# tdj28/ml-depth-pro-video

Measured on AMD Instinct MI355X. Metric: frames/sec at 1536x1536 (1/2/4/8 MI355X) + depth L1 vs reference, higher is better.
Workload: dtype bf16+f16; 1 GPU; BASELINE config 2/3: one 1536x1536 frame per GPU per step through DepthPro.infer (patch+image+FOV ViT-L, decoder, heads), hipGraph replay; global_batch=1, parallelism=frame-dp1, graph=True

## Files before the change

### ml-depth-pro-video_amd/csrc/dp_gemm.hip

```cpp
#include "dp_gemm_impl.h"

namespace dpg {
std::atomic<int> g_dbg_flags{0};

constexpr int DP_MAX_DEV = 64;
std::atomic<int> g_num_cu[DP_MAX_DEV];
int num_cus() {
  int dev = 0;
  if (hipGetDevice(&dev) != hipSuccess || dev < 0) dev = 0;
  std::atomic<int>& slot = g_num_cu[dev < DP_MAX_DEV ? dev : 0];
  int n = slot.load(std::memory_order_relaxed);
  if (n <= 0) {
    if (hipDeviceGetAttribute(&n, hipDeviceAttributeMultiprocessorCount, dev) != hipSuccess || n <= 0) n = 256;
    if (dev < DP_MAX_DEV) slot.store(n, std::memory_order_relaxed);
  }
  return n;
}
}

namespace {
int launch_tile(const GemmP& p, int tile, bool conv, bool bf16, hipStream_t s) {
  switch (tile) {
    case DP_TILE_PBIG_320x256: case DP_TILE_PBIG_256x256: return launch_part_pbig(p, tile, conv, bf16, s);
    case DP_TILE_256x64: case DP_TILE_256x32: case DP_TILE_128x128: case DP_TILE_DUAL_256x128:
      return launch_part_small(p, tile, conv, bf16, s);
    case DP_TILE_8PH_256x256: case DP_TILE_P8PH_256x256: return launch_part_8ph(p, tile, conv, bf16, s);
    case DP_TILE_8PH_320x256: return launch_part_8ph320(p, conv, bf16, s);
    case DP_TILE_CV3_256x256: return launch_part_cv3(p, conv, bf16, s);
    case DP_TILE_CV3_192x256: return launch_part_cv3(p, conv, bf16, s, 12);
    case DP_TILE_CV3_384x128: return launch_part_cv3(p, conv, bf16, s, 24);
    case DP_TILE_BIG_320x256: case DP_TILE_BIG_512x128: return launch_part_big320(p, tile, conv, bf16, s);
    default: return launch_part_big(p, tile, conv, bf16, s);
  }
}
}


extern "C" int dp_gemm_debug_flags(int flags) {
  g_dbg_flags.store(flags, std::memory_order_relaxed);
  return 0;
}

extern "C" int64_t dp_gemm_workspace_size(void) { return SK_FLAG_BYTES + (int64_t)SK_MAX_WG * SK_TILE_F * 4; }

namespace {
__global__ void ws_check_kernel(uint32_t* __restrict__ ws, int32_t* __restrict__ status) {
  const uint32_t err = ws[DP_GEMM_WS_ERROR_OFFSET / 4];
  if (threadIdx.x == 0) status[0] = (int32_t)err;
  if (err == 0) return;
  __syncthreads();
  for (int i = threadIdx.x; i < (int)(SK_FLAG_BYTES / 4); i += blockDim.x) ws[i] = 0u;
}
}

extern "C" int dp_gemm_workspace_check(void* workspace, int32_t* status, dp_stream_t stream) {
  if (!workspace || !status) return DP_ERR_ARG;
  hipLaunchKernelGGL(ws_check_kernel, dim3(1), dim3(256), 0, (hipStream_t)stream, (uint32_t*)workspace, status);
  DP_CHECK_LAUNCH();
  return 0;
}

namespace {
int gemm_plan(const dp_gemm_args* a, GemmP& p, int& tile) {
  if (!a) return DP_ERR_ARG;
  if (a->M <= 0 || a->N <= 0 || a->K <= 0) return DP_ERR_SHAPE;
  if (a->K % BK != 0 || a->N % 4 != 0) return DP_ERR_SHAPE;
  if (a->ldb % 8 != 0 || (a->a_mode == DP_A_DENSE && a->lda % 8 != 0)) return DP_ERR_ALIGN;
  if ((!a->head_w && a->store_mode != DP_STORE_HEAD_PS && a->ldc % 4 != 0) || (a->R1 && a->ldr1 % 4 != 0) ||
      (a->R2 && a->ldr2 % 4 != 0) || (a->pos && a->ldpos % 4 != 0))
    return DP_ERR_ALIGN;
  if (!a->A || !a->B || (!a->C && !a->ln_xl)) return DP_ERR_ARG;
  if (a->dtype != DP_BF16 && a->dtype != DP_F16) return DP_ERR_DTYPE;
  if (a->c_dtype != DP_BF16 && a->c_dtype != DP_F16 && a->c_dtype != DP_F32) return DP_ERR_DTYPE;
  if (a->c_dtype != DP_F32 && a->c_dtype != a->dtype) return DP_ERR_DTYPE;
  if (a->accumulate && a->c_dtype != DP_F32) return DP_ERR_DTYPE;
  if (a->pos && (a->pos_group <= 0)) return DP_ERR_ARG;
  if (a->a_mode == DP_A_CONV) {
    if (a->in_c % BK != 0 || a->k_h * a->k_w * a->in_c != a->K) return DP_ERR_SHAPE;
    if (a->out_h <= 0 || a->out_w <= 0 || a->stride <= 0 || a->M % (a->out_h * a->out_w) != 0)
      return DP_ERR_SHAPE;
  }
  if (a->store_mode == DP_STORE_HEAD_PS) {
    if (a->a_mode != DP_A_CONV || a->N != 128 || !a->head_w || !a->head_corr || a->c_dtype != DP_F32 ||
        a->accumulate || a->R1 || a->R2 || a->pos || a->gamma || a->act != DP_ACT_NONE)
      return DP_ERR_ARG;
  }
  if (a->store_mode == DP_STORE_ROWS && a->head_corr) {
    if (a->a_mode != DP_A_CONV || a->k_h != 3 || a->k_w != 3 || a->pad != 1 || a->stride != 1 || a->head_w ||
        a->relu_a ||
        a->row_group || a->out_h != a->in_h || a->out_w != a->in_w || a->N % 8 != 0 || a->N < 128 ||
        (a->tile != DP_TILE_AUTO && a->tile <= DP_TILE_256x32))
      return DP_ERR_ARG;
  }
  if (a->store_mode == DP_STORE_DECONV2X2) {
    if (a->dc_cout % 4 != 0 || a->N != 4 * a->dc_cout || a->dc_h <= 0 || a->dc_w <= 0 ||
        a->M % (a->dc_h * a->dc_w) != 0)
      return DP_ERR_SHAPE;
  }
  const bool lnp = a->ln_part_out || a->ln_xb_out || a->ln_xl || a->ln_rs_out,
             lnc = a->ln_part_in || a->ln_colsum || a->ln_rs_in;
  if (lnp && lnc) return DP_ERR_ARG;
  if (lnp && !a->ln_xl && (!a->ln_part_out || !a->ln_xb_out || !a->accumulate || !a->C || a->c_dtype != DP_F32 ||
                           a->act != DP_ACT_NONE || a->N % 128 != 0))
    return DP_ERR_ARG;
  if (a->ln_xl && (!a->ln_xb_out || !a->accumulate || a->c_dtype != DP_F32 || a->act != DP_ACT_NONE ||
                   a->N % 128 != 0 || a->ldc % 8 != 0 || (long long)a->M * a->ldc * 4 >= 0xFFFFFF00LL))
    return DP_ERR_ARG;
  if (lnc && (!(a->ln_part_in || a->ln_rs_in) || (a->ln_part_in && a->ln_rs_in) || !a->ln_colsum || a->K != 1024 ||
              a->accumulate || a->c_dtype == DP_F32 || a->gamma || (a->act != DP_ACT_NONE && a->act != DP_ACT_GELU) ||
              !(a->ln_eps > 0.f)))
    return DP_ERR_ARG;
  if (a->ln_rs_out && (!a->ln_xl || !a->ln_part_out || a->N != 1024 || !(a->ln_eps > 0.f) ||
                       !(a->workspace && a->workspace_bytes >= dp_gemm_workspace_size()) ||
                       (a->M + 319) / 320 > 1023 - LN_CNT_WORD))
    return DP_ERR_ARG;
  if (a->ln_rs_in && a->tile != DP_TILE_AUTO && a->tile != DP_TILE_P8PH_256x256) return DP_ERR_ARG;
  if ((lnp || lnc) && a->tile != DP_TILE_AUTO && a->tile != DP_TILE_8PH_320x256 &&
      !(lnc && a->tile == DP_TILE_P8PH_256x256))
    return DP_ERR_ARG;
  const bool ws_ok = a->workspace && a->workspace_bytes >= dp_gemm_workspace_size();
  const int dbg = g_dbg_flags.load(std::memory_order_relaxed);
  tile = a->tile;
  if (a->store_mode == DP_STORE_HEAD_PS) {
    if (tile != DP_TILE_CV3_256x256 && tile != DP_TILE_CV3_384x128 && tile != DP_TILE_BIG_256x128)
      tile = a->M >= 512 * 256 ? DP_TILE_BIG_512x128 : DP_TILE_BIG_256x128;
  } else if (a->head_w) {
    if (a->N > 32 || a->store_mode != DP_STORE_ROWS) return DP_ERR_SHAPE;
    tile = DP_TILE_256x32;
  }
  const bool col8_shape = a->N % 8 == 0 && !(a->store_mode == DP_STORE_DECONV2X2 && a->dc_cout % 8 != 0);
  const bool col8_align = !(a->c_dtype != DP_F32 && a->ldc % 8 != 0) && !(a->R1 && a->ldr1 % 8 != 0) &&
                          !(a->R2 && a->ldr2 % 8 != 0);
  if (tile >= DP_TILE_BIG_256x256) {
    if (!col8_shape) return DP_ERR_SHAPE;
    if (!col8_align) return DP_ERR_ALIGN;
  }
  const long long tiles256 = (long long)((a->M + 255) / 256) * (a->N / 256);
  if (tile == DP_TILE_STREAMK_256x256 && (!ws_ok || a->N % 256 != 0)) return DP_ERR_ARG;
  if (tile == DP_TILE_AUTO) {
    if (a->N <= 32) tile = DP_TILE_256x32;
    else if (a->N <= 64) tile = DP_TILE_256x64;
    else if (!col8_shape || !col8_align) tile = DP_TILE_128x128;
    else if (a->N == 128 && a->M >= 512 * 256) {
      const bool cv3 = a->a_mode == DP_A_CONV && a->k_h == 3 && a->k_w == 3 && a->stride == 1 && a->pad == 1 &&
                       a->in_h == a->in_w && a->out_h == a->in_h && a->out_w == a->in_w && a->in_w % 16 == 0 &&
                       a->in_c % 64 == 0 && a->head_corr && a->store_mode == DP_STORE_ROWS && a->c_dtype != DP_F32 &&
                       !a->R1 && !a->R2 && !a->gamma && !a->pos && !a->accumulate && !a->row_group && !(dbg & 4096);
      tile = !cv3 ? DP_TILE_BIG_512x128
             : a->in_w % 48 == 0 ? DP_TILE_CV3_384x128 : DP_TILE_CV3_256x256;
    }
    else if (a->N % 256 != 0) tile = DP_TILE_BIG_256x128;
    else if (ws_ok && a->a_mode == DP_A_CONV && !(dbg & 32) && tiles256 < num_cus() &&
             a->K >= 4608) {
      tile = DP_TILE_STREAMK_256x256;
    } else if (ws_ok && a->K <= 256 && tiles256 >= 1024) {
      tile = DP_TILE_STREAMK_256x256;
    } else {
      const long long ncu = num_cus();
      const long long tiles320 = (long long)((a->M + 319) / 320) * (a->N / 256);
      const long long tiles128 = (long long)((a->M + 255) / 256) * (a->N / 128);
      const long long cost256 = (tiles256 + ncu - 1) / ncu * 256 * 20, cost320 = (tiles320 + ncu - 1) / ncu * 320 * 20;
      const long long cost128 = (tiles128 + ncu - 1) / ncu * 128 * 23;
      if (cost128 < cost256 && cost128 < cost320) tile = DP_TILE_BIG_256x128;
      else if (cost320 < cost256) tile = DP_TILE_BIG_320x256;
      else tile = (tiles256 >= 600 && a->a_mode != DP_A_CONV) ? DP_TILE_8PH_256x256 : DP_TILE_BIG_256x256;
      if (tile == DP_TILE_8PH_256x256 && (dbg & 8192)) tile = DP_TILE_BIG_320x256;
      else if (tile == DP_TILE_8PH_256x256 && (dbg & 16384)) tile = DP_TILE_BIG_256x256;
    }
  }
  int ksplit = 1;
  if (tile == DP_TILE_SPLITK_256x256) {
    if (!ws_ok || a->N % 256 != 0 || a->store_mode != DP_STORE_ROWS || a->row_group || a->head_w || a->head_corr ||
        lnp || lnc)
      return DP_ERR_ARG;
    const long long ncu = num_cus(), kt = a->K / BK;
    const long long slab = (long long)a->M * a->N * 4;
    long long sp = ncu / tiles256;
    if (sp > kt / 2) sp = kt / 2;
    if (sp > (a->workspace_bytes - SK_FLAG_BYTES) / slab) sp = (a->workspace_bytes - SK_FLAG_BYTES) / slab;
    if (sp > 32) sp = 32;
    if (sp < 2) return DP_ERR_SHAPE;
    ksplit = (int)sp;
  }
  unsigned c_bytes = 0;
  if (a->store_mode == DP_STORE_ROWS && !a->head_w && !a->head_corr) {
    long long last = a->M - 1;
    if (a->row_group) last = (last / a->row_group) * a->row_group_out + a->row_off + last % a->row_group;
    const long long ext = (last * a->ldc + a->N) * (a->c_dtype == DP_F32 ? 4 : 2);
    if (ext < 0xFFFFFF00LL) c_bytes = (unsigned)ext;
  }
  unsigned dcv_bytes = 0;
  if (a->store_mode == DP_STORE_DECONV2X2 && a->c_dtype != DP_F32) {
    const long long ext = ((4LL * a->M - 1) * a->ldc + a->dc_cout) * 2;
    if (ext < 0xFFFFFF00LL) dcv_bytes = (unsigned)ext;
  }
  const bool off32 = (a->a_mode != DP_A_DENSE || (long long)a->M * a->lda < (1LL << 31)) &&
                     (long long)a->N * a->ldb < (1LL << 31);
  if (!off32) c_bytes = dcv_bytes = 0;
  if ((tile == DP_TILE_PBIG_320x256 || tile == DP_TILE_PBIG_256x256) && (!c_bytes || a->N % 256)) return DP_ERR_ARG;
  if (a->tile == DP_TILE_AUTO && c_bytes && !(dbg & 1024)) {
    const long long ncu = num_cus();
    const bool dense_ok = a->a_mode == DP_A_CONV || (dbg & 2048);
    if (dense_ok && tile == DP_TILE_BIG_320x256 && (long long)((a->M + 319) / 320) * (a->N / 256) >= 2 * ncu)
      tile = DP_TILE_PBIG_320x256;
    else if (dense_ok && tile == DP_TILE_BIG_256x256 && tiles256 >= 2 * ncu)
      tile = DP_TILE_PBIG_256x256;
  }
  const bool dcv = a->store_mode == DP_STORE_DECONV2X2 && !a->relu_a && !a->gamma && a->act == DP_ACT_NONE &&
                   a->dc_w >= 8;
  if (a->tile == DP_TILE_AUTO && dcv && col8_shape && col8_align && !(dbg & (1 << 23)) && tiles256 >= 128)
    tile = DP_TILE_P8PH_256x256;
  if (tile == DP_TILE_P8PH_256x256 || (a->tile == DP_TILE_AUTO && tile == DP_TILE_8PH_256x256 && !(dbg & (1 << 22)))) {
    const bool ok = a->a_mode == DP_A_DENSE && a->N % 256 == 0 && a->K >= 128 && a->c_dtype != DP_F32 &&
                    ((a->store_mode == DP_STORE_ROWS && c_bytes) || (dcv && dcv_bytes)) && !a->R1 && !a->R2 && !a->pos && !a->accumulate &&
                    !a->row_group && !a->head_w && !a->head_corr && !(dbg & (1 << 20));
    if (tile == DP_TILE_P8PH_256x256 && !ok) return DP_ERR_ARG;
    if (ok) tile = DP_TILE_P8PH_256x256;
    if (ok && dcv) c_bytes = dcv_bytes;
  }
  const bool lnc_p8 = lnc && tile == DP_TILE_P8PH_256x256 && (ws_ok || a->ln_rs_in) && !(dbg & (1 << 25)) &&
                      (a->ln_rs_in || (long long)(a->M + 255) / 256 * 256 * 8 <= (long long)SK_TILE_F * 4);
  if (a->ln_rs_in && !lnc_p8) return DP_ERR_ARG;
  if ((lnp || lnc) && !lnc_p8) tile = DP_TILE_8PH_320x256;
  if (tile == DP_TILE_8PH_320x256 || (a->tile == DP_TILE_AUTO && tile == DP_TILE_BIG_320x256 && !(dbg & (1 << 15)))) {
    const bool plain = a->a_mode == DP_A_DENSE && !a->relu_a && a->N % 256 == 0 && a->store_mode == DP_STORE_ROWS &&
                       !a->R1 && !a->R2 && !a->pos && !a->row_group && !a->head_w && !a->head_corr &&
                       !(dbg & (1 << 20)) && off32;
    const bool epi_ok = (!a->accumulate && a->c_dtype != DP_F32) ||
                        (a->accumulate && a->c_dtype == DP_F32 && a->act == DP_ACT_NONE);
    if (tile == DP_TILE_8PH_320x256 && !(plain && epi_ok)) return DP_ERR_ARG;
    if (plain && epi_ok) tile = DP_TILE_8PH_320x256;
  }
  if (a->tile == DP_TILE_AUTO && !(dbg & (1 << 16)) && a->a_mode == DP_A_CONV && a->k_h == 3 && a->k_w == 3 &&
      a->stride == 1 && a->pad == 1 && a->in_h == a->in_w && a->out_h == a->in_h && a->out_w == a->in_w &&
      a->in_w % 16 == 0 && a->in_c % 64 == 0 && a->N % 256 == 0 && a->store_mode == DP_STORE_ROWS &&
      !a->row_group && !a->head_w && !a->head_corr && (long long)a->M * a->in_c < (1LL << 30) && off32 &&
      a->c_dtype != DP_F32 && !a->gamma && !a->pos && !a->accumulate && a->act != DP_ACT_GELU && col8_align &&
      (long long)(a->M / 256) * (a->N / 256) >= 4LL * num_cus())
    tile = DP_TILE_CV3_256x256;
  else if (a->tile == DP_TILE_AUTO && !(dbg & (1 << 16)) && a->a_mode == DP_A_CONV &&
           a->k_h == 3 && a->k_w == 3 && a->stride == 1 && a->pad == 1 && a->in_h == a->in_w &&
           a->out_h == a->in_h && a->out_w == a->in_w && a->in_w % 16 == 0 && a->in_w % 12 == 0 &&
           a->in_c % 64 == 0 && a->N % 256 == 0 && a->store_mode == DP_STORE_ROWS && !a->row_group && !a->head_w &&
           !a->head_corr && (long long)a->M * a->in_c < (1LL << 30) && off32 && a->c_dtype != DP_F32 && !a->gamma &&
           !a->pos && !a->accumulate && a->act != DP_ACT_GELU && col8_align) {
    const long long t12 = (long long)(a->M / ((long long)a->in_w * a->in_w)) * (a->in_w / 12) * (a->in_w / 16) * (a->N / 256);
    const long long ncu = num_cus();
    if (t12 >= 2 * ncu && t12 % ncu == 0 && ((long long)(a->M / 256) * (a->N / 256)) % ncu != 0) tile = DP_TILE_CV3_192x256;
    else if (t12 <= ncu && 2 * t12 >= ncu) tile = DP_TILE_CV3_192x256;
  }
  if (tile >= DP_TILE_BIG_256x256 && !col8_shape) return DP_ERR_SHAPE;
  if (tile >= DP_TILE_BIG_256x256 && !col8_align) return DP_ERR_ALIGN;
  if (tile == DP_TILE_CV3_256x256 || tile == DP_TILE_CV3_192x256 || tile == DP_TILE_CV3_384x128) {
    const int th = tile == DP_TILE_CV3_192x256 ? 12 : tile == DP_TILE_CV3_384x128 ? 24 : 16, S = a->out_w;
    const bool hps = a->store_mode == DP_STORE_HEAD_PS, bc = a->store_mode == DP_STORE_ROWS && a->head_corr;
    if (a->a_mode != DP_A_CONV || a->k_h != 3 || a->k_w != 3 || a->stride != 1 || a->pad != 1 || a->in_h != S ||
        a->in_w != S || a->out_h != S || S % 16 != 0 || S % th != 0 || a->row_group || (a->head_w && !hps) || a->gamma ||
        a->pos || a->accumulate || (a->act != DP_ACT_NONE && a->act != DP_ACT_RELU) ||
        (long long)a->M * a->in_c >= (1LL << 30) || (long long)a->N * a->ldb >= (1LL << 31))
      return DP_ERR_ARG;
    if (!hps && a->store_mode != DP_STORE_ROWS) return DP_ERR_ARG;
    if (bc && (a->c_dtype == DP_F32 || a->R1 || a->R2 || a->N % 128 != 0)) return DP_ERR_ARG;
    if (!hps && !bc && (a->c_dtype == DP_F32 || a->N % 256 != 0)) return DP_ERR_ARG;
    if (th == 12 && (hps || bc)) return DP_ERR_ARG;
    if (th == 24 && !((hps || bc) && a->N == 128)) return DP_ERR_ARG;
  }
  if (a->store_mode == DP_STORE_ROWS && a->head_corr && tile != DP_TILE_BIG_512x128 && tile != DP_TILE_CV3_256x256 &&
      tile != DP_TILE_CV3_384x128)
    return DP_ERR_ARG;
  if (tile == DP_TILE_CV3_384x128 && (!a->head_corr || a->N != 128)) return DP_ERR_ARG;

  p.M = a->M; p.N = a->N; p.K = a->K;
  p.A = (const u16*)a->A; p.lda = a->lda;
  p.B = (const u16*)a->B; p.ldb = a->ldb;
  p.relu_a = a->relu_a;
  p.in_h = a->in_h; p.in_w = a->in_w; p.in_c = a->in_c; p.k_h = a->k_h; p.k_w = a->k_w;
  p.stride = a->stride; p.pad = a->pad; p.out_h = a->out_h; p.out_w = a->out_w;
  p.bias = a->bias; p.act = a->act; p.gamma = a->gamma;
  p.pos = a->pos; p.ldpos = a->ldpos; p.pos_group = a->pos_group; p.pos_off = a->pos_off;
  p.R1 = (const u16*)a->R1; p.ldr1 = a->ldr1; p.R2 = (const u16*)a->R2; p.ldr2 = a->ldr2;
  p.C = a->C; p.ldc = a->ldc; p.c_dtype = a->c_dtype; p.accumulate = a->accumulate;
  p.store_mode = a->store_mode; p.dc_h = a->dc_h; p.dc_w = a->dc_w; p.dc_cout = a->dc_cout;
  p.row_group = a->row_group; p.row_group_out = a->row_group_out; p.row_off = a->row_off;
  p.head_w = a->head_w; p.head_b = a->head_b; p.head_corr = a->head_corr;
  p.ln_part_out = a->ln_part_out; p.ln_xb_out = (u16*)a->ln_xb_out; p.ln_xl = (u16*)a->ln_xl;
  p.ln_part_in = a->ln_part_in; p.ln_colsum = a->ln_colsum; p.ln_eps = a->ln_eps;
  p.ln_rs = a->ln_rs_in;
  p.ln_rs_out = a->ln_rs_out;
  p.ln_cnt = a->ln_rs_out ? (unsigned*)a->workspace + LN_CNT_WORD : nullptr;
  p.tiles_n = 1;
  p.tiles_m = 1;
  if (tile == DP_TILE_STREAMK_256x256) {
    p.tiles_n = a->N / 256;
    p.tiles_m = (a->M + 255) / 256;
  }
  p.dbg = dbg;
  p.c_bytes = c_bytes;
  p.ksplit = ksplit;
  p.kpart = ksplit > 1 ? (float*)((char*)a->workspace + SK_FLAG_BYTES) : nullptr;
  p.groups = 1;
  return 0;
}
}

extern "C" int dp_gemm_plan(const dp_gemm_args* a, int32_t* tile_out, int32_t* grid_out) {
  GemmP p;
  int tile = 0;
  const int rc = gemm_plan(a, p, tile);
  if (rc) return rc;
  const int N = a->N, M = a->M;
  int bm = 256, bn = 128;
  switch (tile) {
    case DP_TILE_256x64: bn = 64; break;
    case DP_TILE_256x32: bn = 32; break;
    case DP_TILE_128x128: bm = 128; bn = 128; break;
    case DP_TILE_BIG_256x128: case DP_TILE_BIG_256x128_K32: case DP_TILE_DEEP_256x128: bn = 128; break;
    case DP_TILE_BIG_320x256: bm = 320; bn = 256; break;
    case DP_TILE_BIG_512x128: bm = 512; bn = 128; break;
    case DP_TILE_DUAL_256x128: bn = 128; break;
    case DP_TILE_PBIG_320x256: case DP_TILE_8PH_320x256: bm = 320; bn = 256; break;
    case DP_TILE_CV3_192x256: bm = 192; bn = 256; break;
    case DP_TILE_CV3_384x128: bm = 384; bn = 128; break;
    default: bn = 256;
  }
  if (tile_out) *tile_out = tile;
  int grid = ((M + bm - 1) / bm) * ((N + bn - 1) / bn);
  if (tile == DP_TILE_PBIG_320x256 || tile == DP_TILE_PBIG_256x256 || tile == DP_TILE_P8PH_256x256)
    grid = grid < num_cus() ? grid : num_cus();
  if (tile == DP_TILE_SPLITK_256x256) grid *= p.ksplit;
  if (grid_out) *grid_out = tile == DP_TILE_STREAMK_256x256 ? sk_grid(p) : grid;
  return 0;
}

extern "C" int dp_gemm(const dp_gemm_args* a, dp_stream_t stream) {
  GemmP p;
  int tile = 0;
  const int rc = gemm_plan(a, p, tile);
  if (rc) return rc;
  hipStream_t s = (hipStream_t)stream;
  const bool conv = a->a_mode == DP_A_CONV;
  if (tile == DP_TILE_STREAMK_256x256) return launch_part_sk(p, conv, a->workspace, a->dtype == DP_BF16, s);
  if (tile == DP_TILE_SPLITK_256x256) return launch_part_splitk(p, conv, a->dtype == DP_BF16, s);
  if (tile == DP_TILE_P8PH_256x256 && a->ln_part_in && !a->ln_rs_in) {
    float* rs = (float*)((char*)a->workspace + SK_FLAG_BYTES);
    hipLaunchKernelGGL(ln_merge_kernel, dim3((a->M + 255) / 256), dim3(256), 0, s, a->ln_part_in, a->M, a->ln_eps, rs);
    DP_CHECK_LAUNCH();
    p.ln_rs = rs;
  }
  return launch_tile(p, tile, conv, a->dtype == DP_BF16, s);
}

extern "C" int dp_gemm_grouped(const dp_gemm_args* a, int32_t groups, dp_stream_t stream) {
  if (!a || groups < 1 || groups > DP_MAX_GROUPS) return DP_ERR_ARG;
  if (groups == 1) return dp_gemm(a, stream);
  GemmP p;
  for (int g = 0; g < groups; ++g) {
    GemmP q;
    int t = 0;
    const int rc = gemm_plan(&a[g], q, t);
    if (rc) return rc;
    const dp_gemm_args &x = a[0], &y = a[g];
    if (y.M != x.M || y.N != x.N || y.K != x.K || y.dtype != x.dtype || y.lda != x.lda || y.ldb != x.ldb ||
        y.a_mode != DP_A_DENSE || x.a_mode != DP_A_DENSE || y.relu_a || y.act != x.act ||
        !y.bias != !x.bias || !y.gamma != !x.gamma || !y.pos != !x.pos || y.ldpos != x.ldpos ||
        y.pos_group != x.pos_group || y.pos_off != x.pos_off || !y.R1 != !x.R1 || y.ldr1 != x.ldr1 ||
        !y.R2 != !x.R2 || y.ldr2 != x.ldr2 || y.ldc != x.ldc || y.c_dtype != x.c_dtype ||
        y.accumulate != x.accumulate || y.store_mode != DP_STORE_ROWS || x.store_mode != DP_STORE_ROWS ||
        y.row_group != x.row_group || y.row_group_out != x.row_group_out || y.row_off != x.row_off ||
        y.head_w || y.head_corr || y.N % 8 != 0 || y.ln_part_out || y.ln_xb_out || y.ln_xl || y.ln_part_in ||
        y.ln_rs_out || y.ln_rs_in ||
        y.ln_colsum)
      return DP_ERR_ARG;
    if (g == 0) p = q;
    p.grp[g] = GemmP::Group{q.A, q.B, q.bias, q.gamma, q.pos, q.R1, q.R2, q.C};
  }
  p.groups = groups;
  hipStream_t s = (hipStream_t)stream;
  return launch_part_big(p, TILE_GRP_128x128, false, a->dtype == DP_BF16, s);
}
```

### ml-depth-pro-video_amd/csrc/dp_gemm_cv3.hip

```cpp
#include "dp_gemm_impl.h"

namespace {

constexpr int CV_TW = 16;
constexpr int CV_PW = CV_TW + 2;
template <int TH> struct CvGeo {
  static constexpr int PIX = (TH + 2) * CV_PW;
  static constexpr int PPW = (PIX * 8 + 511) / 512;
  static constexpr int PATCH_B = 8 * PPW * 1024;
  static constexpr int FM = TH / 2, HQ = FM / 2;
  static constexpr int NREAL = (PIX + 7) / 8;
  static constexpr bool TIGHT = NREAL * 1024 + ((FM + 1) * CV_PW + 2) * 128 < 65536;
  static constexpr int PSTRIDE = TIGHT ? NREAL * 1024 : PATCH_B;
  static constexpr int TRASH = 2 * PSTRIDE;
  static constexpr int WOFF = TIGHT ? 2 * PSTRIDE + 1024 : 2 * PATCH_B;
};

constexpr int CV_EPI_RES = 0, CV_EPI_BC = 1, CV_EPI_HPS = 2;
constexpr int CV_STAMPS = 10, CV_STAMP_WGS = 4096;
__device__ unsigned long long g_cv3_stamp[CV_STAMP_WGS * CV_STAMPS];
template <typename K_, bool RELU, int BN, int EPI, int ABL = 0, int TH = 16>
__global__ void __launch_bounds__(512, 1) gemm_cv3_kernel(const GemmP p) {
  using G = CvGeo<TH>;
  constexpr int FM = G::FM, HQ = G::HQ, PPW = G::PPW, CV_PATCH_B = G::PATCH_B, CV_PIX = G::PIX;
  constexpr bool TIGHT = G::TIGHT;
  constexpr int PSTRIDE = G::PSTRIDE, WOFF = G::WOFF;
  constexpr int TN = BN / 4, FN = TN / 16, QF = FN / 2;
  static_assert(TH == 16 || TH == 12 || (TH == 24 && BN == 128), "tile rows");
  constexpr int NBH = BN / 128;
  constexpr int B_B = BN * 128;
  static_assert(EPI != CV_EPI_RES || BN == 256, "residual epilogue: BN 256");
  static_assert(EPI != CV_EPI_HPS || BN == 128, "head epilogue: one parity (32 columns) per wave");
  __shared__ __attribute__((aligned(1024))) char smem[WOFF + 2 * B_B];

  const int tid = threadIdx.x, lane = tid & 63;
  const int wave = tid >> 6;
  const int wave_u = __builtin_amdgcn_readfirstlane(wave);
  unsigned long long st_[CV_STAMPS] = {};
  if constexpr ((ABL & 8) != 0) { st_[0] = __builtin_amdgcn_s_memtime(); st_[4] = __builtin_amdgcn_s_memrealtime(); }
  const int wm = wave >> 2, wn = wave & 3;
  const int nwg = gridDim.x, bid = blockIdx.x;
  const int xcd = bid & 7, q8 = nwg >> 3, r8 = nwg & 7;
  const int wgid = (xcd < r8 ? xcd * (q8 + 1) : r8 * (q8 + 1) + (xcd - r8) * q8) + (bid >> 3);
  const int S = p.out_w, tpr = S / CV_TW, tpi = (S / TH) * tpr;
  const int tn = wgid % p.tiles_n, sp = wgid / p.tiles_n;
  const int img = sp / tpi, r_ = sp - img * tpi;
  const int y0 = (r_ / tpr) * TH, x0 = (r_ % tpr) * CV_TW, n0 = tn * BN;
  const int cin = p.in_c, CB = cin / 64;
  const int KT = CB * 9;

  constexpr uint32_t CV_PAD = 0x80000000u;
  auto patch_off = [&](int i, int c0) __attribute__((always_inline)) {
    const int c = c0 + i * 64;
    const int P = c >> 3, slot = c & 7;
    uint32_t off = CV_PAD;
    if (P < CV_PIX) {
      const int pr = P / CV_PW, pc = P - pr * CV_PW;
      const int iy = y0 - 1 + pr, ix = x0 - 1 + pc;
      if ((unsigned)iy < (unsigned)S && (unsigned)ix < (unsigned)S)
        off = 2u * (uint32_t)(((img * S + iy) * S + ix) * cin + ((slot ^ (P & 7)) << 3));
    }
    return off;
  };
  const uint32_t lds0 = __builtin_amdgcn_readfirstlane(lds_addr(smem));
  const u32x4_t a_rs = raw_rsrc(p.A, (uint32_t)((long long)p.M * cin * 2));

  constexpr int HALF = 128 * 128;
  const int prow = wave * 8 + (lane >> 3);
  const int pchunk = (lane & 7) ^ ((lane >> 3) & 7);
  const uint32_t boff = 2u * (uint32_t)((n0 + prow) * (int)p.ldb + pchunk * 8);
  auto issue_b = [&](int h, int t) {
    const uint32_t dst = lds0 + WOFF + (t & 1) * B_B + h * HALF + wave_u * 1024;
    #pragma unroll
    for (int i = 0; i < 2; ++i) glds16s(boff, p.B + (long long)(h * 128 + i * 64) * p.ldb + 64 * t, dst + i * 8192);
  };
  auto issue_patch3 = [&](int cb, int buf, int i0) {
    int c0 = wave * PPW * 64 + lane;
    asm volatile("" : "+v"(c0));
    #pragma unroll
    for (int i = i0; i < i0 + PPW / 2; ++i) {
      const int j = wave_u * PPW + i;
      const uint32_t dst = lds0 + ((!TIGHT || j < G::NREAL) ? buf * PSTRIDE + j * 1024 : G::TRASH);
      glds16b(patch_off(i, c0) + cb * 128, a_rs, dst);
    }
  };

  f32x4_t acc[FM][FN];
  #pragma unroll
  for (int i = 0; i < FM; ++i)
    #pragma unroll
    for (int j = 0; j < FN; ++j) acc[i][j] = f32x4_t{0.f, 0.f, 0.f, 0.f};
  const int frow = lane & 15, fchunk = lane >> 4;
  uint4 af[2][HQ], bf[2][2][QF];
  typedef __attribute__((address_space(3))) const char lds_c;
  typedef __attribute__((address_space(3))) const u32x4_t lds_u4;
  uint32_t abase[8][2], bbase[2];
  {
    const int PB = wm * FM * CV_PW + frow;
    #pragma unroll
    for (int v = 0; v < 8; ++v)
      #pragma unroll
      for (int ks = 0; ks < 2; ++ks) abase[v][ks] = lds0 + PB * 128 + (((ks * 4 + fchunk) ^ ((PB + v) & 7)) << 4);
    #pragma unroll
    for (int ks = 0; ks < 2; ++ks)
      bbase[ks] = lds0 + WOFF + (wn * TN + frow) * 128 + (((ks * 4 + fchunk) ^ (frow & 7)) << 4);
  }
  auto readA = [&](int qm, int ky, int kx, int pb) __attribute__((always_inline)) {
    const int boff_ = TIGHT ? pb * PSTRIDE : 0;
    #pragma unroll
    for (int ks = 0; ks < 2; ++ks)
      #pragma unroll
      for (int fm = 0; fm < HQ; ++fm) {
        const int c = (qm * HQ + fm + ky) * CV_PW + kx;
        af[ks][fm] = __builtin_bit_cast(uint4, *(lds_u4*)((lds_c*)(uintptr_t)abase[c & 7][ks] + boff_ + c * 128));
      }
    if constexpr (RELU && (ABL & 32)) {
      #pragma unroll
      for (int ks = 0; ks < 2; ++ks)
        #pragma unroll
        for (int fm = 0; fm < HQ; ++fm) af[ks][fm] = relu_pk16(af[ks][fm]);
      __builtin_amdgcn_sched_barrier(0);
    }
  };
  auto readB = [&](int qn, int st) __attribute__((always_inline)) {
    #pragma unroll
    for (int ks = 0; ks < 2; ++ks)
      #pragma unroll
      for (int fn = 0; fn < QF; ++fn)
        bf[qn][ks][fn] = __builtin_bit_cast(uint4, *(lds_u4*)((lds_c*)(uintptr_t)bbase[ks] + st * B_B + (qn * (TN / 2) + fn * 16) * 128));
  };
  auto tick = [&]() -> unsigned long long {
    if constexpr ((ABL & 256) != 0) return __builtin_amdgcn_s_memtime();
    return 0ull;
  };
  auto mma = [&](int qm, int qn) {
    const unsigned long long m0_ = tick();
    asm volatile("s_waitcnt lgkmcnt(0)" ::: "memory");
    __builtin_amdgcn_sched_barrier(0);
    const unsigned long long m1_ = tick();
    if constexpr ((ABL & 256) != 0) st_[8] += m1_ - m0_;
    if constexpr (ABL & 4) return;
    if constexpr (RELU && !(ABL & 32)) {
      if (qn == 0) {
        #pragma unroll
        for (int ks = 0; ks < 2; ++ks)
          #pragma unroll
          for (int fm = 0; fm < HQ; ++fm) af[ks][fm] = relu_pk16(af[ks][fm]);
      }
    }
    if constexpr ((ABL & 1536) == 0) __builtin_amdgcn_s_setprio(1);
    #pragma unroll
    for (int ks = 0; ks < 2; ++ks)
      #pragma unroll
      for (int fm = 0; fm < HQ; ++fm) {
        #pragma unroll
        for (int fn = 0; fn < QF; ++fn)
          acc[qm * HQ + fm][qn * QF + fn] = K_::mfma16(bf[qn][ks][fn], af[ks][fm], acc[qm * HQ + fm][qn * QF + fn]);
      }
    if constexpr ((ABL & 1536) == 0) __builtin_amdgcn_s_setprio(0);
    if constexpr ((ABL & 256) != 0) { __builtin_amdgcn_sched_barrier(0); st_[9] += tick() - m1_; }
  };
  auto bar = [&]() {
    const unsigned long long b0_ = tick();
    if constexpr ((ABL & 16) == 0) asm volatile("s_barrier" ::: "memory");
    if constexpr ((ABL & 256) != 0) st_[7] += tick() - b0_;
  };

  issue_patch3(0, 0, 0); issue_patch3(0, 0, PPW / 2);
  #pragma unroll
  for (int h = 0; h < NBH; ++h) issue_b(h, 0);
  if (KT > 1) {
    #pragma unroll
    for (int h = 0; h < NBH; ++h) issue_b(h, 1);
    wait_vmcnt<2 * NBH>();
  } else {
    wait_vmcnt<0>();
  }
  lds_barrier();
  if constexpr ((ABL & 8) != 0) st_[1] = __builtin_amdgcn_s_memtime();
  if constexpr ((ABL & 512) != 0) { if (wave_u >= 4) __builtin_amdgcn_s_setprio(1); }
  if (wm == 1) bar();
  int cb = 0;
  auto block = [&](auto st0_tag) __attribute__((always_inline)) {
    constexpr int ST0 = decltype(st0_tag)::value;
    constexpr int pb = ST0;
    const bool nb = cb + 1 < CB;
    #pragma unroll
    for (int tap = 0; tap < 9; ++tap) {
      const int ky = tap / 3, kx = tap - ky * 3, st = (ST0 + tap) & 1;
      const int t = cb * 9 + tap;
      const bool np = tap == 0 && nb;
      const bool n2 = t + 2 < KT;
      readA(0, ky, kx, pb); readB(0, st); readB(1, st);
      if (np && !(ABL & 2) && !(ABL & 128)) { issue_patch3(cb + 1, pb ^ 1, 0); issue_patch3(cb + 1, pb ^ 1, PPW / 2); }
      bar(); mma(0, 0); mma(0, 1); bar();
      readA(1, ky, kx, pb);
      if (n2 && !(ABL & 2) && !(ABL & 64)) issue_b(0, t + 2);
      const unsigned long long v0_ = tick();
      if (np) { if (n2) wait_vmcnt<PPW + 2>(); else wait_vmcnt<PPW>(); }
      else { if (n2) wait_vmcnt<2>(); else wait_vmcnt<0>(); }
      if constexpr ((ABL & 256) != 0) st_[6] += tick() - v0_;
      if (NBH == 2 && n2 && !(ABL & 2) && !(ABL & 64)) issue_b(1, t + 2);
      bar(); mma(1, 0); mma(1, 1); bar();
    }
    if constexpr (!TIGHT) {
      const uint32_t d = pb ? (uint32_t)-CV_PATCH_B : (uint32_t)CV_PATCH_B;
      #pragma unroll
      for (int v = 0; v < 8; ++v)
        #pragma unroll
        for (int ks = 0; ks < 2; ++ks) abase[v][ks] += d;
    }
    ++cb;
  };
  for (int pair = 0; pair < CB / 2; ++pair) {
    block(std::integral_constant<int, 0>{});
    block(std::integral_constant<int, 1>{});
  }
  if (CB & 1) block(std::integral_constant<int, 0>{});
  if (wm == 0) bar();
  if constexpr ((ABL & 512) != 0) __builtin_amdgcn_s_setprio(0);

  lds_barrier();
  if constexpr ((ABL & 8) != 0) st_[2] = __builtin_amdgcn_s_memtime();
  if constexpr ((ABL & 1) != 0) {
    float z = 0.f;
    #pragma unroll
    for (int i = 0; i < FM; ++i)
      #pragma unroll
      for (int j = 0; j < FN; ++j) z += acc[i][j][0];
    if (z == 1234.5f) ((float*)p.C)[tid] = z;
    return;
  }
  const int t = lane & 15, g = lane >> 4;
  const int nw = n0 + wn * TN;
  f32x4_t bias[FN];
  #pragma unroll
  for (int fn = 0; fn < FN; ++fn)
    bias[fn] = p.bias ? *(const f32x4_t*)(p.bias + nw + fn * 16 + 4 * g) : f32x4_t{0.f, 0.f, 0.f, 0.f};
  auto mrow = [&](int fm) { return (long long)((img * S + y0 + wm * FM + fm) * S + x0); };
  if constexpr (EPI == CV_EPI_HPS) {
    const int q = nw >> 5, dy = q >> 1, dx = q & 1;
    float hw[FN][4];
    #pragma unroll
    for (int fn = 0; fn < FN; ++fn)
      #pragma unroll
      for (int r = 0; r < 4; ++r) hw[fn][r] = p.head_w[(nw & 31) + fn * 16 + 4 * g + r];
    const long long W2 = 2LL * S;
    #pragma unroll 1
    for (int fm = 0; fm < FM; ++fm) {
      const int y = y0 + wm * FM + fm, x = x0 + t;
      float z[FN][4];
      #pragma unroll
      for (int fn = 0; fn < FN; ++fn)
        #pragma unroll
        for (int r = 0; r < 4; ++r) z[fn][r] = acc[fm][fn][r] + bias[fn][r];
      const bool top = y == 0 && dy == 0, bot = y == S - 1 && dy == 1;
      const bool lft = x == 0 && dx == 0, rgt = x == S - 1 && dx == 1;
      if (top || bot || lft || rgt) {
        #pragma unroll
        for (int a = 0; a < 3; ++a)
          #pragma unroll
          for (int c = 0; c < 3; ++c) {
            const bool oob = (a == 0 && top) || (a == 2 && bot) || (c == 0 && lft) || (c == 2 && rgt);
            if (oob) {
              #pragma unroll
              for (int fn = 0; fn < FN; ++fn)
                #pragma unroll
                for (int r = 0; r < 4; ++r) z[fn][r] -= p.head_corr[(a * 3 + c) * 32 + (nw & 31) + fn * 16 + 4 * g + r];
            }
          }
      }
      float hs = 0.f;
      #pragma unroll
      for (int fn = 0; fn < FN; ++fn)
        #pragma unroll
        for (int r = 0; r < 4; ++r) hs += fmaxf(z[fn][r], 0.f) * hw[fn][r];
      hs += __shfl_xor(hs, 16);
      hs += __shfl_xor(hs, 32);
      if (g == 0) ((float*)p.C)[((long long)img * 2 * S + 2 * y + dy) * W2 + 2 * x + dx] = fmaxf(hs + p.head_b, 0.f);
    }
  } else {
    constexpr int CH = TN / 8, RPI = 64 / CH;
    char* slab = smem + wave * (16 * TN * 2);
    constexpr int PD = 4;
    uint2 rb1[PD][FN], rb2[PD][FN];
    auto loadr = [&](int fm, uint2 (&r1)[FN], uint2 (&r2)[FN]) __attribute__((always_inline)) {
      if constexpr (EPI == CV_EPI_RES) {
        const long long m = mrow(fm) + t;
        #pragma unroll
        for (int fn = 0; fn < FN; ++fn) {
          const int col = nw + fn * 16 + 4 * g;
          if (p.R1) r1[fn] = *(const uint2*)(p.R1 + m * p.ldr1 + col);
          if (p.R2) r2[fn] = *(const uint2*)(p.R2 + m * p.ldr2 + col);
        }
      }
    };
    auto addr = [&](f32x4_t& x, uint2 r) __attribute__((always_inline)) {
      x[0] += K_::to_f(r.x & 0xffff); x[1] += K_::to_f(r.x >> 16);
      x[2] += K_::to_f(r.y & 0xffff); x[3] += K_::to_f(r.y >> 16);
    };
    #pragma unroll
    for (int i = 0; i < PD; ++i) loadr(i, rb1[i], rb2[i]);
    #pragma unroll
    for (int fm = 0; fm < FM; ++fm) {
      uint2 (&r1c)[FN] = rb1[fm % PD];
      uint2 (&r2c)[FN] = rb2[fm % PD];
      const int y = y0 + wm * FM + fm, x = x0 + t;
      const bool border = y == 0 || y == S - 1 || x == 0 || x == S - 1;
      #pragma unroll
      for (int fn = 0; fn < FN; ++fn) {
        f32x4_t xv = acc[fm][fn] + bias[fn];
        if constexpr (EPI == CV_EPI_BC) {
          if (border) {
            #pragma unroll 1
            for (int tp = 0; tp < 9; ++tp) {
              const int a = tp / 3, c = tp - 3 * (tp / 3);
              const bool oob = (a == 0 && y == 0) || (a == 2 && y == S - 1) || (c == 0 && x == 0) || (c == 2 && x == S - 1);
              if (oob) xv -= *(const f32x4_t*)(p.head_corr + tp * p.N + nw + fn * 16 + 4 * g);
            }
          }
        }
        if (p.act == DP_ACT_RELU) {
          #pragma unroll
          for (int r = 0; r < 4; ++r) xv[r] = fmaxf(xv[r], 0.f);
        }
        if constexpr (EPI == CV_EPI_RES) {
          if (p.R1) addr(xv, r1c[fn]);
          if (p.R2) addr(xv, r2c[fn]);
        }
        const int chunk = fn * 2 + (g >> 1);
        uint2 w;
        w.x = K_::pack2(xv[0], xv[1]);
        w.y = K_::pack2(xv[2], xv[3]);
        *(uint2*)(slab + t * (TN * 2) + ((chunk ^ (t & (CH - 1))) << 4) + (g & 1) * 8) = w;
      }
      #pragma unroll
      for (int k = 0; k < 16 / RPI; ++k) {
        const int row = k * RPI + lane / CH, chunk = lane % CH;
        const uint4 d = *(const uint4*)(slab + row * (TN * 2) + ((chunk ^ (row & (CH - 1))) << 4));
        *(uint4*)((u16*)p.C + (mrow(fm) + row) * p.ldc + nw + chunk * 8) = d;
      }
      if (fm + PD < FM) loadr(fm + PD, r1c, r2c);
    }
  }
  if constexpr ((ABL & 8) != 0) {
    asm volatile("s_waitcnt vmcnt(0)" ::: "memory");
    st_[3] = __builtin_amdgcn_s_memtime();
    st_[5] = __builtin_amdgcn_s_memrealtime();
    if (tid == 0 && blockIdx.x < CV_STAMP_WGS) {
      #pragma unroll
      for (int k = 0; k < CV_STAMPS; ++k) g_cv3_stamp[blockIdx.x * CV_STAMPS + k] = st_[k];
    }
  }
}

template <typename K_>
int launch_cv3(const GemmP& p0, hipStream_t s, int th) {
  GemmP p = p0;
  const int S = p.out_w;
  if (p.k_h != 3 || p.k_w != 3 || p.stride != 1 || p.pad != 1 || p.in_h != S || p.in_w != S || p.out_h != S ||
      S % CV_TW || S % th || p.in_c % 64 || p.M % (S * S) || p.row_group || (p.head_w && p.store_mode != DP_STORE_HEAD_PS) ||
      p.gamma || p.pos || p.accumulate || (p.act != DP_ACT_NONE && p.act != DP_ACT_RELU))
    return DP_ERR_ARG;
  if ((long long)p.M * p.in_c >= (1LL << 30) || (long long)p.N * p.ldb >= (1LL << 31)) return DP_ERR_ARG;
  int epi, bn;
  if (p.store_mode == DP_STORE_HEAD_PS) {
    if (p.N != 128 || !p.head_w || !p.head_corr || p.c_dtype != DP_F32 || p.R1 || p.R2 || p.act) return DP_ERR_ARG;
    epi = CV_EPI_HPS; bn = 128;
  } else if (p.store_mode == DP_STORE_ROWS && p.head_corr) {
    if (p.c_dtype == DP_F32 || p.R1 || p.R2 || p.N % 128) return DP_ERR_ARG;
    epi = CV_EPI_BC; bn = p.N % 256 ? 128 : 256;
  } else if (p.store_mode == DP_STORE_ROWS) {
    if (p.c_dtype == DP_F32 || p.N % 256) return DP_ERR_ARG;
    epi = CV_EPI_RES; bn = 256;
  } else {
    return DP_ERR_ARG;
  }
  if (th == 12 && epi != CV_EPI_RES) return DP_ERR_ARG;
  if (th == 24 && ((epi != CV_EPI_BC && epi != CV_EPI_HPS) || bn != 128)) return DP_ERR_ARG;
  p.tiles_n = p.N / bn;
  p.tiles_m = (p.M / (S * S)) * (S / th) * (S / CV_TW);
  dim3 grid(p.tiles_m * p.tiles_n);
  const int abl = (p.dbg & (1 << 24)) ? p.dbg & 2047 : 0;
  if (th == 24) {
    if (epi == CV_EPI_HPS) hipLaunchKernelGGL((gemm_cv3_kernel<K_, false, 128, CV_EPI_HPS, 0, 24>), grid, dim3(512), 0, s, p);
    else if (p.relu_a) hipLaunchKernelGGL((gemm_cv3_kernel<K_, true, 128, CV_EPI_BC, 0, 24>), grid, dim3(512), 0, s, p);
    else hipLaunchKernelGGL((gemm_cv3_kernel<K_, false, 128, CV_EPI_BC, 0, 24>), grid, dim3(512), 0, s, p);
    DP_CHECK_LAUNCH();
    return 0;
  }
  if (th == 12) {
    if (abl == 8 && p.relu_a) hipLaunchKernelGGL((gemm_cv3_kernel<K_, true, 256, CV_EPI_RES, 8, 12>), grid, dim3(512), 0, s, p);
    else if (abl == 1032 && p.relu_a) hipLaunchKernelGGL((gemm_cv3_kernel<K_, true, 256, CV_EPI_RES, 1032, 12>), grid, dim3(512), 0, s, p);
    else if (abl == 520 && p.relu_a) hipLaunchKernelGGL((gemm_cv3_kernel<K_, true, 256, CV_EPI_RES, 520, 12>), grid, dim3(512), 0, s, p);
    else if (abl == 264 && p.relu_a) hipLaunchKernelGGL((gemm_cv3_kernel<K_, true, 256, CV_EPI_RES, 264, 12>), grid, dim3(512), 0, s, p);
    else if (p.relu_a) hipLaunchKernelGGL((gemm_cv3_kernel<K_, true, 256, CV_EPI_RES, 0, 12>), grid, dim3(512), 0, s, p);
    else hipLaunchKernelGGL((gemm_cv3_kernel<K_, false, 256, CV_EPI_RES, 0, 12>), grid, dim3(512), 0, s, p);
    DP_CHECK_LAUNCH();
    return 0;
  }
#define DP_CV3(B_, E_) do { \
    if (p.relu_a) hipLaunchKernelGGL((gemm_cv3_kernel<K_, true, B_, E_>), grid, dim3(512), 0, s, p); \
    else hipLaunchKernelGGL((gemm_cv3_kernel<K_, false, B_, E_>), grid, dim3(512), 0, s, p); } while (0)
  if (epi == CV_EPI_RES && abl && p.relu_a) {
    switch (abl) {
#define DP_CV3A(A_) case A_: hipLaunchKernelGGL((gemm_cv3_kernel<K_, true, 256, CV_EPI_RES, A_>), grid, dim3(512), 0, s, p); break;
      DP_CV3A(1) DP_CV3A(2) DP_CV3A(3) DP_CV3A(4) DP_CV3A(5) DP_CV3A(6) DP_CV3A(7) DP_CV3A(8)
      DP_CV3A(10) DP_CV3A(12) DP_CV3A(14) DP_CV3A(24) DP_CV3A(26) DP_CV3A(28) DP_CV3A(30) DP_CV3A(40) DP_CV3A(72)
      DP_CV3A(136) DP_CV3A(264) DP_CV3A(520) DP_CV3A(1032)
#undef DP_CV3A
      default: DP_CV3(256, CV_EPI_RES);
    }
  } else if (epi == CV_EPI_RES) DP_CV3(256, CV_EPI_RES);
  else if (epi == CV_EPI_HPS) DP_CV3(128, CV_EPI_HPS);
  else if (bn == 256) DP_CV3(256, CV_EPI_BC);
  else DP_CV3(128, CV_EPI_BC);
#undef DP_CV3
  DP_CHECK_LAUNCH();
  return 0;
}

}

extern "C" int dp_cv3_stamps(unsigned long long* dst, int n_wg) {
  if (n_wg > CV_STAMP_WGS) n_wg = CV_STAMP_WGS;
  return (int)hipMemcpyFromSymbol(dst, HIP_SYMBOL(g_cv3_stamp), (size_t)n_wg * CV_STAMPS * 8, 0, hipMemcpyDeviceToHost);
}

namespace dpg {
int launch_part_cv3(const GemmP& p, bool conv, bool bf16, hipStream_t s, int th) {
  if (!conv) return DP_ERR_ARG;
  return bf16 ? launch_cv3<KBF16>(p, s, th) : launch_cv3<KF16>(p, s, th);
}
}
```

Baseline: 52.66 frames/sec.

## Spread next-patch prefetch across taps and apply ReLU before the barrier in cv3 conv

The 3x3 conv kernel used to issue the whole next channel-block patch prefetch at tap 0. It now issues one patch load per tap over the first PPW taps and waits on fewer outstanding loads, which spreads memory traffic and shortens the tap-0 stall. The ReLU on A fragments moves out of the MFMA routine into a separate step placed before each barrier, and the cv3 auto-selection gets a guard so the 32-bit buffer offsets cannot overflow. More profiling stamp slots and ablation variants are added, and the per-tap vmcnt accounting must stay correct for each PPW or the pipeline risks races.

```diff
diff --git a/ml-depth-pro-video_amd/csrc/dp_gemm.hip b/ml-depth-pro-video_amd/csrc/dp_gemm.hip
--- a/ml-depth-pro-video_amd/csrc/dp_gemm.hip
+++ b/ml-depth-pro-video_amd/csrc/dp_gemm.hip
@@ -145,7 +145,8 @@
       const bool cv3 = a->a_mode == DP_A_CONV && a->k_h == 3 && a->k_w == 3 && a->stride == 1 && a->pad == 1 &&
                        a->in_h == a->in_w && a->out_h == a->in_h && a->out_w == a->in_w && a->in_w % 16 == 0 &&
                        a->in_c % 64 == 0 && a->head_corr && a->store_mode == DP_STORE_ROWS && a->c_dtype != DP_F32 &&
-                       !a->R1 && !a->R2 && !a->gamma && !a->pos && !a->accumulate && !a->row_group && !(dbg & 4096);
+                       !a->R1 && !a->R2 && !a->gamma && !a->pos && !a->accumulate && !a->row_group && !(dbg & 4096) &&
+                       (long long)a->M * a->in_c < (1LL << 30);
       tile = !cv3 ? DP_TILE_BIG_512x128
              : a->in_w % 48 == 0 ? DP_TILE_CV3_384x128 : DP_TILE_CV3_256x256;
     }
diff --git a/ml-depth-pro-video_amd/csrc/dp_gemm_cv3.hip b/ml-depth-pro-video_amd/csrc/dp_gemm_cv3.hip
--- a/ml-depth-pro-video_amd/csrc/dp_gemm_cv3.hip
+++ b/ml-depth-pro-video_amd/csrc/dp_gemm_cv3.hip
@@ -17,7 +17,7 @@
 };
 
 constexpr int CV_EPI_RES = 0, CV_EPI_BC = 1, CV_EPI_HPS = 2;
-constexpr int CV_STAMPS = 10, CV_STAMP_WGS = 4096;
+constexpr int CV_STAMPS = 16, CV_STAMP_WGS = 4096;
 __device__ unsigned long long g_cv3_stamp[CV_STAMP_WGS * CV_STAMPS];
 template <typename K_, bool RELU, int BN, int EPI, int ABL = 0, int TH = 16>
 __global__ void __launch_bounds__(512, 1) gemm_cv3_kernel(const GemmP p) {
@@ -74,6 +74,13 @@
     #pragma unroll
     for (int i = 0; i < 2; ++i) glds16s(boff, p.B + (long long)(h * 128 + i * 64) * p.ldb + 64 * t, dst + i * 8192);
   };
+  auto issue_patch1 = [&](int cb, int buf, int i) {
+    int c0 = wave * PPW * 64 + lane;
+    asm volatile("" : "+v"(c0));
+    const int j = wave_u * PPW + i;
+    const uint32_t dst = lds0 + ((!TIGHT || j < G::NREAL) ? buf * PSTRIDE + j * 1024 : G::TRASH);
+    glds16b(patch_off(i, c0) + cb * 128, a_rs, dst);
+  };
   auto issue_patch3 = [&](int cb, int buf, int i0) {
     int c0 = wave * PPW * 64 + lane;
     asm volatile("" : "+v"(c0));
@@ -129,6 +136,7 @@
       for (int fn = 0; fn < QF; ++fn)
         bf[qn][ks][fn] = __builtin_bit_cast(uint4, *(lds_u4*)((lds_c*)(uintptr_t)bbase[ks] + st * B_B + (qn * (TN / 2) + fn * 16) * 128));
   };
+  int so_ = 0;
   auto tick = [&]() -> unsigned long long {
     if constexpr ((ABL & 256) != 0) return __builtin_amdgcn_s_memtime();
     return 0ull;
@@ -138,16 +146,8 @@
     asm volatile("s_waitcnt lgkmcnt(0)" ::: "memory");
     __builtin_amdgcn_sched_barrier(0);
     const unsigned long long m1_ = tick();
-    if constexpr ((ABL & 256) != 0) st_[8] += m1_ - m0_;
+    if constexpr ((ABL & 256) != 0) st_[8 + so_] += m1_ - m0_;
     if constexpr (ABL & 4) return;
-    if constexpr (RELU && !(ABL & 32)) {
-      if (qn == 0) {
-        #pragma unroll
-        for (int ks = 0; ks < 2; ++ks)
-          #pragma unroll
-          for (int fm = 0; fm < HQ; ++fm) af[ks][fm] = relu_pk16(af[ks][fm]);
-      }
-    }
     if constexpr ((ABL & 1536) == 0) __builtin_amdgcn_s_setprio(1);
     #pragma unroll
     for (int ks = 0; ks < 2; ++ks)
@@ -158,12 +158,22 @@
           acc[qm * HQ + fm][qn * QF + fn] = K_::mfma16(bf[qn][ks][fn], af[ks][fm], acc[qm * HQ + fm][qn * QF + fn]);
       }
     if constexpr ((ABL & 1536) == 0) __builtin_amdgcn_s_setprio(0);
-    if constexpr ((ABL & 256) != 0) { __builtin_amdgcn_sched_barrier(0); st_[9] += tick() - m1_; }
+    if constexpr ((ABL & 256) != 0) { __builtin_amdgcn_sched_barrier(0); st_[9 + so_] += tick() - m1_; }
+  };
+  auto relu_early = [&]() __attribute__((always_inline)) {
+    if constexpr (RELU && !(ABL & 32)) {
+      __builtin_amdgcn_sched_barrier(0);
+      #pragma unroll
+      for (int ks = 0; ks < 2; ++ks)
+        #pragma unroll
+        for (int fm = 0; fm < HQ; ++fm) af[ks][fm] = relu_pk16(af[ks][fm]);
+      __builtin_amdgcn_sched_barrier(0);
+    }
   };
   auto bar = [&]() {
     const unsigned long long b0_ = tick();
     if constexpr ((ABL & 16) == 0) asm volatile("s_barrier" ::: "memory");
-    if constexpr ((ABL & 256) != 0) st_[7] += tick() - b0_;
+    if constexpr ((ABL & 256) != 0) st_[7 + so_] += tick() - b0_;
   };
 
   issue_patch3(0, 0, 0); issue_patch3(0, 0, PPW / 2);
@@ -189,19 +199,24 @@
     for (int tap = 0; tap < 9; ++tap) {
       const int ky = tap / 3, kx = tap - ky * 3, st = (ST0 + tap) & 1;
       const int t = cb * 9 + tap;
-      const bool np = tap == 0 && nb;
+      const bool np = tap < PPW && nb;
       const bool n2 = t + 2 < KT;
+      if constexpr ((ABL & 256) != 0) so_ = tap == 0 ? 4 : 0;
+      const unsigned long long s0_ = tick();
       readA(0, ky, kx, pb); readB(0, st); readB(1, st);
-      if (np && !(ABL & 2) && !(ABL & 128)) { issue_patch3(cb + 1, pb ^ 1, 0); issue_patch3(cb + 1, pb ^ 1, PPW / 2); }
+      if (np && !(ABL & 2) && !(ABL & 128)) issue_patch1(cb + 1, pb ^ 1, tap);
+      relu_early();
       bar(); mma(0, 0); mma(0, 1); bar();
       readA(1, ky, kx, pb);
       if (n2 && !(ABL & 2) && !(ABL & 64)) issue_b(0, t + 2);
+      relu_early();
       const unsigned long long v0_ = tick();
-      if (np) { if (n2) wait_vmcnt<PPW + 2>(); else wait_vmcnt<PPW>(); }
+      if (np) { if (n2) wait_vmcnt<1 + 2>(); else wait_vmcnt<1>(); }
       else { if (n2) wait_vmcnt<2>(); else wait_vmcnt<0>(); }
-      if constexpr ((ABL & 256) != 0) st_[6] += tick() - v0_;
+      if constexpr ((ABL & 256) != 0) st_[6 + so_] += tick() - v0_;
       if (NBH == 2 && n2 && !(ABL & 2) && !(ABL & 64)) issue_b(1, t + 2);
       bar(); mma(1, 0); mma(1, 1); bar();
+      if constexpr ((ABL & 256) != 0) st_[tap == 0 ? 15 : 14] += tick() - s0_;
     }
     if constexpr (!TIGHT) {
       const uint32_t d = pb ? (uint32_t)-CV_PATCH_B : (uint32_t)CV_PATCH_B;
@@ -383,7 +398,9 @@
   dim3 grid(p.tiles_m * p.tiles_n);
   const int abl = (p.dbg & (1 << 24)) ? p.dbg & 2047 : 0;
   if (th == 24) {
-    if (epi == CV_EPI_HPS) hipLaunchKernelGGL((gemm_cv3_kernel<K_, false, 128, CV_EPI_HPS, 0, 24>), grid, dim3(512), 0, s, p);
+    if (epi == CV_EPI_BC && !p.relu_a && abl == 8) hipLaunchKernelGGL((gemm_cv3_kernel<K_, false, 128, CV_EPI_BC, 8, 24>), grid, dim3(512), 0, s, p);
+    else if (epi == CV_EPI_BC && !p.relu_a && abl == 264) hipLaunchKernelGGL((gemm_cv3_kernel<K_, false, 128, CV_EPI_BC, 264, 24>), grid, dim3(512), 0, s, p);
+    else if (epi == CV_EPI_HPS) hipLaunchKernelGGL((gemm_cv3_kernel<K_, false, 128, CV_EPI_HPS, 0, 24>), grid, dim3(512), 0, s, p);
     else if (p.relu_a) hipLaunchKernelGGL((gemm_cv3_kernel<K_, true, 128, CV_EPI_BC, 0, 24>), grid, dim3(512), 0, s, p);
     else hipLaunchKernelGGL((gemm_cv3_kernel<K_, false, 128, CV_EPI_BC, 0, 24>), grid, dim3(512), 0, s, p);
     DP_CHECK_LAUNCH();
```

Measured after the change: 53.27 frames/sec (median of 6 runs). 1.01x the previous value.
